# aehogan/lammps-induced-dipole-polarization-pair-style

Measured on AMD Instinct MI355X. Metric: atom-steps/sec, higher is better.
Workload: dtype f64

## Files before the change

lammps-induced-dipole-polarization-pair-style_amd/csrc/lab/api_env_knobs.inc:

```
  if (const char *e = getenv("POLAR_ABLATE")) h->ablate = atoi(e);
  if (const char *e = getenv("POLAR_HOST_COLORS")) h->host_colors = atoi(e) != 0;
  if (const char *e = getenv("POLAR_SWEEP_KERNEL")) h->sweep_kernel = atoi(e);
  if (const char *e = getenv("POLAR_TILE_WAVES")) h->tile_waves = atoi(e) == 8 ? 8 : 4;
  if (const char *e = getenv("POLAR_TILE_WIDE")) h->tile_wide = atoi(e) != 0;
  if (const char *e = getenv("POLAR_CACHE_R2")) h->cache_r2 = atoi(e);
  if (const char *e = getenv("POLAR_LJ_TYPED")) h->lj_typed = atoi(e) != 0;
  if (const char *e = getenv("POLAR_STATIC_XQ")) h->static_xq = atoi(e) != 0;
  if (const char *e = getenv("POLAR_POL_FIRST")) h->pol_first = atoi(e) != 0;
  if (const char *e = getenv("POLAR_LP_WG_PER_CU")) h->lp_wg_per_cu = atoi(e);
  if (const char *e = getenv("POLAR_LP_QM")) h->lp_quad_major = atoi(e) != 0;
  if (const char *e = getenv("POLAR_LP_TILES")) h->lp_tiles = atoi(e) == 1 ? 1 : 2;
  if (const char *e = getenv("POLAR_LP_ROWS")) h->lp_rows = std::max(1, std::min(64, atoi(e)));
  if (const char *e = getenv("POLAR_LP_PAIRS")) h->lp_pairs = atoi(e) != 0;
  if (const char *e = getenv("POLAR_CLUSTER_DIST")) h->cluster_dist = atof(e);
  if (const char *e = getenv("POLAR_CLUSTER_MAX")) h->cluster_max = std::max(1, std::min(4, atoi(e)));
  if (const char *e = getenv("POLAR_LP_DEPTH")) { int v = atoi(e); h->lp_depth = (v == 2 || v == 3) ? v : 0; }
  if (const char *e = getenv("POLAR_QUAD_BLOCK")) { int v = atoi(e); if (v >= 64 && v <= 1024 && v % 64 == 0) h->quad_block = v; }
  if (const char *e = getenv("POLAR_FIELD_BLOCK")) { int v = atoi(e); if (v >= 64 && v <= 1024 && v % 64 == 0) h->field_block = v; }
  if (const char *e = getenv("POLAR_FORCE_LITERAL")) h->force_literal = atoi(e) != 0;
```

lammps-induced-dipole-polarization-pair-style_amd/csrc/polar_api.hip:

```cpp
#include "polar_handle.hpp"

namespace {
void upload_types(polar_handle *h, int ntypes, const double *const t[7]) {
  need_device(h);
  const size_t m = (size_t)(ntypes + 1) * (ntypes + 1);
  std::vector<double> pack(8 * m, 0.0);
  for (size_t k = 0; k < m; k++) {
    pack[8 * k + 0] = t[6][k]; pack[8 * k + 1] = t[5][k]; pack[8 * k + 2] = t[0][k]; pack[8 * k + 3] = t[1][k];
    pack[8 * k + 4] = t[2][k]; pack[8 * k + 5] = t[3][k]; pack[8 * k + 6] = t[4][k];
  }
  h->d_lj.ensure(8 * m);
  HIPCHECK(hipMemcpy(h->d_lj.p, pack.data(), 8 * m * sizeof(double), hipMemcpyHostToDevice));
  h->P.ntypes = ntypes;
  h->P.ljpack = h->d_lj.p;
  h->ntypes = ntypes;
  h->types_set = true;
}

void upload_coul(polar_handle *h, double g_ewald, double qqrd2e, const double *slj, const double *scoul, int nbits,
                 int mask, int shift, double tabinnersq, const double *const t[8]) {
  need_device(h);
  h->P.g_ewald = g_ewald; h->P.qqrd2e = qqrd2e;
  for (int k = 0; k < 4; k++) { h->P.special_lj[k] = slj[k]; h->P.special_coul[k] = scoul[k]; }
  h->P.ncoultablebits = nbits; h->P.ncoulmask = mask; h->P.ncoulshiftbits = shift; h->P.tabinnersq = tabinnersq;
// ... 222 lines not shown

const char *polar_last_error(const polar_handle *h) { return h ? h->err.c_str() : "null handle"; }
const char *polar_last_warning(const polar_handle *h) { return h ? h->warn.c_str() : ""; }

int polar_pair_settings(polar_handle *h, int narg, const char *const *arg) {
  return guarded(h, [&]() { h->ph.settings(narg, arg); h->colors_valid = false; h->nl_pitch = h->dd_pitch = 0; h->cl_pitch = 0; h->un_pitch = 0; h->pitch16 = 0; return POLAR_OK; });
}
int polar_pair_coeff(polar_handle *h, int ntypes, int narg, const char *const *arg) {
  return guarded(h, [&]() { h->ph.coeff(ntypes, narg, arg); return POLAR_OK; });
}
int polar_pair_modify(polar_handle *h, int narg, const char *const *arg) {
  return guarded(h, [&]() { h->ph.modify(narg, arg); return POLAR_OK; });
}
int polar_pair_init(polar_handle *h, double g_ewald, double qqrd2e, const double special_lj[4],
                    const double special_coul[4]) {
  return guarded(h, [&]() {
    PairHost &p = h->ph;
    p.init(g_ewald, qqrd2e, special_lj, special_coul);
    h->coul_set = false;
    if (h->have_device) {
      HIPCHECK(hipSetDevice(h->device));
      const double *t[7] = {p.lj1.data(), p.lj2.data(), p.lj3.data(), p.lj4.data(), p.offset.data(), p.cut_ljsq.data(), p.cutsq.data()};
      upload_types(h, p.ntypes, t);
      if (p.ncoultablebits == 0) {
        const double *c[8];
        double dummy = 0.0;
        for (int k = 0; k < 8; k++) c[k] = &dummy;
        upload_coul(h, g_ewald, qqrd2e, special_lj, special_coul, 0, 0, 0, 0.0, c);
      }
    }
    return POLAR_OK;
  });
}
double polar_pair_cut(const polar_handle *h, int i, int j) {
  if (!h || !h->ph.inited || i < 1 || j < 1 || i > h->ph.ntypes || j > h->ph.ntypes) return -1.0;
  return std::sqrt(h->ph.cutsq[(size_t)i * h->ph.w() + j]);
}
double polar_pair_single(const polar_handle *h, double qi, double qj, int itype, int jtype, double rsq,
                         double factor_coul, double factor_lj, double *fforce) {
  double ff = 0.0, e;
  try {
    e = h->ph.single(qi, qj, itype, jtype, rsq, factor_coul, factor_lj, ff);
  } catch (const std::exception &ex) {
    const_cast<polar_handle *>(h)->err = ex.what();
    e = ff = std::nan("");
  }
  if (fforce) *fforce = ff;
  return e;
}
const void *polar_pair_extract(const polar_handle *h, const char *name, int *dim) {
  if (!h || !name) return nullptr;
  if (dim) *dim = 0;
  if (strcmp(name, "cut_coul") == 0) return &h->ph.st.cut_coul;
  if (dim) *dim = 2;
  if (strcmp(name, "epsilon") == 0) return h->ph.epsilon.data();
  if (strcmp(name, "sigma") == 0) return h->ph.sigma.data();
  if (strcmp(name, "cut_lj") == 0) return h->ph.cut_lj.data();
  return nullptr;
}
int polar_get_settings(const polar_handle *h, polar_settings *out) {
  if (!h || !out) return POLAR_ERR_STATE;
  *out = h->ph.st;
  return POLAR_OK;
}
namespace {
const int kRestartMagic = 0x524C4F50;
const int kRestartVersion = 2;
const int kRestartPayloadV1 = 4 * (int)sizeof(double) + 10 * (int)sizeof(int);
const int kRestartPayload = kRestartPayloadV1 + 4 * (int)sizeof(int) + (int)sizeof(double);
}
int polar_restart_pack(const polar_handle *h, void *buf, int max_bytes) {
  if (!h) return POLAR_ERR_STATE;
  const int total = POLAR_RESTART_HEADER_BYTES + kRestartPayload;
  if (!buf) return total;
  if (max_bytes < total) return POLAR_ERR_INPUT;
  const polar_settings &st = h->ph.st;
  char *p = (char *)buf;
  const int head[3] = {kRestartMagic, kRestartVersion, kRestartPayload};
  memcpy(p, head, sizeof(head)); p += sizeof(head);
  const double d[4] = {st.polar_precision, st.polar_damp, st.polar_gamma, st.dd_cutoff};
  memcpy(p, d, sizeof(d)); p += sizeof(d);
  const int iv[10] = {st.iterations_max, st.damping_type, st.zodid, st.fixed_iteration, st.polar_gs, st.polar_gs_ranked,
                      st.use_previous, st.debug, st.device_neigh, st.restart_polar};
  memcpy(p, iv, sizeof(iv)); p += sizeof(iv);
  const int iv2[4] = {st.deterministic, st.rccl_halo, st.polar_accel, 0};
  memcpy(p, iv2, sizeof(iv2)); p += sizeof(iv2);
  memcpy(p, &st.polar_sor, sizeof(double));
  return total;
}
int polar_restart_unpack(polar_handle *h, const void *buf, int nbytes) {
  return guarded(h, [&]() {
    if (!buf || nbytes < POLAR_RESTART_HEADER_BYTES) throw InputError("not a polarization restart record");
    const char *p = (const char *)buf;
    int head[3];
    memcpy(head, p, sizeof(head)); p += sizeof(head);
    if (head[0] != kRestartMagic) throw InputError("not a polarization restart record");
    const bool v1 = head[1] == 1 && head[2] == kRestartPayloadV1, v2 = head[1] == kRestartVersion && head[2] == kRestartPayload;
    if (!(v1 || v2) || nbytes < POLAR_RESTART_HEADER_BYTES + head[2])
      throw InputError("polarization restart record of an unknown version or length");
    double d[4]; int iv[10];
    memcpy(d, p, sizeof(d)); p += sizeof(d);
    memcpy(iv, p, sizeof(iv)); p += sizeof(iv);
    polar_settings s = h->ph.st;
    s.polar_precision = d[0]; s.polar_damp = d[1]; s.polar_gamma = d[2]; s.dd_cutoff = d[3];
    s.iterations_max = iv[0]; s.damping_type = iv[1]; s.zodid = iv[2]; s.fixed_iteration = iv[3]; s.polar_gs = iv[4];
    s.polar_gs_ranked = iv[5]; s.use_previous = iv[6]; s.debug = iv[7]; s.device_neigh = iv[8]; s.restart_polar = iv[9];
// ... 676 lines not shown
```

lammps-induced-dipole-polarization-pair-style_amd/csrc/polar_common.hpp:

```cpp
#pragma once

#include <hip/hip_runtime.h>
#include <stdint.h>

#ifdef POLAR_LAB
#define POLAR_LAB_PARAM , int ablate
#define POLAR_LAB_PASS , ablate
#define POLAR_ABL(bit) (ablate & (bit))
#else
#define POLAR_LAB_PARAM
#define POLAR_LAB_PASS
#define POLAR_ABL(bit) 0
#endif

namespace polar {


struct __attribute__((aligned(64))) AtomRec {
  double x, mx;
  double y, my;
  double z, mz;
  double q, a;
};

// ... 121 lines not shown
__device__ __forceinline__ double quad_xor(double v, const int which) {
  int lo = __double2loint(v), hi = __double2hiint(v);
  if (which == 1) {
    lo = __builtin_amdgcn_update_dpp(0, lo, 0xB1, 0xF, 0xF, true);
    hi = __builtin_amdgcn_update_dpp(0, hi, 0xB1, 0xF, 0xF, true);
  } else {
    lo = __builtin_amdgcn_update_dpp(0, lo, 0x4E, 0xF, 0xF, true);
    hi = __builtin_amdgcn_update_dpp(0, hi, 0x4E, 0xF, 0xF, true);
  }
  return __hiloint2double(hi, lo);
}
__device__ __forceinline__ double quad_sum(double v) {
  v += quad_xor(v, 1);
  v += quad_xor(v, 2);
  return v;
}

struct RowList {
  const int *cnt;
  long long pitch;
};
__device__ __forceinline__ void row_range(const RowList &L, int i, long long &beg, long long &end) {
  beg = (long long)i * L.pitch;
  const long long c = L.cnt[i];
  end = beg + (c < L.pitch ? c : L.pitch);
}

__device__ __forceinline__ void min_image_rint(const Box &b, double xi, double yi, double zi, double xj, double yj,
                                               double zj, double &dx, double &dy, double &dz) {
  double ex = xi - xj, ey = yi - yj, ez = zi - zj;
  const double nz = b.periodic[2] ? rint(ez * b.inv[2]) : 0.0;
  ez = fma(-b.prd[2], nz, ez); ey = fma(-b.yz, nz, ey); ex = fma(-b.xz, nz, ex);
  const double ny = b.periodic[1] ? rint(ey * b.inv[1]) : 0.0;
  ey = fma(-b.prd[1], ny, ey); ex = fma(-b.xy, ny, ex);
  const double nx = b.periodic[0] ? rint(ex * b.inv[0]) : 0.0;
  ex = fma(-b.prd[0], nx, ex);
  dx = ex; dy = ey; dz = ez;
}
template <bool TRI>
__device__ __forceinline__ bool min_image_rint_w(const Box &b, double xi, double yi, double zi, double xj, double yj,
                                                 double zj, double &dx, double &dy, double &dz) {
  double ex = xi - xj, ey = yi - yj, ez = zi - zj;
  const double nz = b.periodic[2] ? rint(ez * b.inv[2]) : 0.0;
  ez = fma(-b.prd[2], nz, ez);
  if (TRI) { ey = fma(-b.yz, nz, ey); ex = fma(-b.xz, nz, ex); }
  const double ny = b.periodic[1] ? rint(ey * b.inv[1]) : 0.0;
  ey = fma(-b.prd[1], ny, ey);
  if (TRI) ex = fma(-b.xy, ny, ex);
  const double nx = b.periodic[0] ? rint(ex * b.inv[0]) : 0.0;
  ex = fma(-b.prd[0], nx, ex);
  dx = ex; dy = ey; dz = ez;
  return nz != 0.0 || ny != 0.0 || nx != 0.0;
}
__host__ __device__ __forceinline__ void frac_coords(const Box &b, const double lo[3], double x, double y, double z, double fr[3]) {
  fr[2] = (z - lo[2]) * b.inv[2];
  if (b.triclinic) {
    fr[1] = ((y - lo[1]) - b.yz * fr[2] * 1.0) * b.inv[1];
    fr[0] = ((x - lo[0]) - b.xy * fr[1] - b.xz * fr[2]) * b.inv[0];
  } else {
    fr[1] = (y - lo[1]) * b.inv[1];
    fr[0] = (x - lo[0]) * b.inv[0];
  }
}
template <bool EXACT>
__device__ __forceinline__ void pair_del(const Box &b, double xi, double yi, double zi, double xj, double yj,
                                         double zj, double &dx, double &dy, double &dz) {
  if (EXACT) min_image_del(b, xi, yi, zi, xj, yj, zj, dx, dy, dz);
  else min_image_rint(b, xi, yi, zi, xj, yj, zj, dx, dy, dz);
}

__host__ __device__ __forceinline__ long long lp_slot(long long e, int qm = 1) {
  const long long p = e & 63;
  const long long lane = qm ? (((p & 15) << 2) | (p >> 4)) : p;
  return ((e >> 8) << 8) + (lane << 2) + ((e >> 6) & 3);
}

#define POLAR_NL_SAMEMOL 0x40000000
#define POLAR_NL_MASK 0x3FFFFFFF

struct RecQuad { double2 a, b, c, d; };
__device__ __forceinline__ RecQuad fetch_records(const AtomRec *__restrict__ rec, int j, double2 *stage, int lane) {
  const int q4 = lane >> 2;
  const char *base = reinterpret_cast<const char *>(rec);
  const unsigned piece = (unsigned)(lane & 3) * 16u, k = lane & 3;
  const unsigned j0 = __shfl(j, q4, 64), j1 = __shfl(j, 16 + q4, 64), j2 = __shfl(j, 32 + q4, 64), j3 = __shfl(j, 48 + q4, 64);
  const double2 p0 = *reinterpret_cast<const double2 *>(base + ((j0 << 6) + piece));
  const double2 p1 = *reinterpret_cast<const double2 *>(base + ((j1 << 6) + piece));
  const double2 p2 = *reinterpret_cast<const double2 *>(base + ((j2 << 6) + piece));
  const double2 p3 = *reinterpret_cast<const double2 *>(base + ((j3 << 6) + piece));
  stage[q4 * 5 + k] = p0; stage[(16 + q4) * 5 + k] = p1;
  stage[(32 + q4) * 5 + k] = p2; stage[(48 + q4) * 5 + k] = p3;
  __builtin_amdgcn_fence(__ATOMIC_RELEASE, "wavefront");
  __builtin_amdgcn_wave_barrier();
  __builtin_amdgcn_fence(__ATOMIC_ACQUIRE, "wavefront");
  RecQuad r;
  r.a = stage[lane * 5]; r.b = stage[lane * 5 + 1]; r.c = stage[lane * 5 + 2]; r.d = stage[lane * 5 + 3];
  __builtin_amdgcn_wave_barrier();
  return r;
}

struct XQ { double2 a, b; };
__device__ __forceinline__ XQ fetch_xq(const double4 *__restrict__ xq, int j, double2 *stage, int lane) {
  const int h2 = lane >> 1;
  const char *base = reinterpret_cast<const char *>(xq);
  const unsigned piece = (unsigned)(lane & 1) * 16u, k = lane & 1;
  const unsigned j0 = __shfl(j, h2, 64), j1 = __shfl(j, 32 + h2, 64);
  const double2 p0 = *reinterpret_cast<const double2 *>(base + ((j0 << 5) + piece));
  const double2 p1 = *reinterpret_cast<const double2 *>(base + ((j1 << 5) + piece));
  stage[h2 * 3 + k] = p0; stage[(32 + h2) * 3 + k] = p1;
  __builtin_amdgcn_fence(__ATOMIC_RELEASE, "wavefront");
  __builtin_amdgcn_wave_barrier();
  __builtin_amdgcn_fence(__ATOMIC_ACQUIRE, "wavefront");
  XQ r;
  r.a = stage[lane * 3]; r.b = stage[lane * 3 + 1];
  __builtin_amdgcn_wave_barrier();
  return r;
}

struct ExpCoef {
  double log2e, ln2hi, ln2lo;
  double c[14];
};
inline ExpCoef make_expcoef() {
  ExpCoef K;
  K.log2e = 1.4426950408889634074; K.ln2hi = 6.93147180369123816490e-01; K.ln2lo = 1.90821492927058770002e-10;
  const double c[14] = {1.0, 1.0, 0.5, 0.16666666666666666, 0.041666666666666664, 0.008333333333333333, 0.001388888888888889, 0.0001984126984126984, 2.48015873015873e-05, 2.7557319223985893e-06, 2.755731922398589e-07, 2.505210838544172e-08, 2.08767569878681e-09, 1.6059043836821613e-10};
  for (int k = 0; k < 14; k++) K.c[k] = c[k];
// ... 91 lines not shown
```

lammps-induced-dipole-polarization-pair-style_amd/csrc/polar_handle.hpp:

```cpp
#pragma once
#include <hip/hip_runtime.h>

#include <algorithm>
#include <initializer_list>
#include <utility>
#include <chrono>
#include <cmath>
#include <cstdio>
#include <cstdlib>
#include <exception>
#include <cstring>
#include <numeric>
#include <string>
#include <thread>
#include <mutex>
#include <condition_variable>
#include <functional>
#include <memory>
#include <stdexcept>
#include <unistd.h>
#include <vector>

#include "pair_host.hpp"
#include "polar_kernels.hpp"
// ... 145 lines not shown
  DBuf<double> d_mu0;
  bool mu0_saved = false;
  int attempt = 0;
  int last_sweeps = 0;
  bool mu_host_in_sync = false;
  std::vector<int> color_off;
  std::vector<int> color_sub;
  int color_nsub = 1;
  DBuf<int> d_bflag; int bflag_n = 0;
  std::vector<int *> h_nl_stage; std::vector<hipEvent_t> ev_nl;
  hipStream_t up_stream = nullptr; hipEvent_t ev_list_up = nullptr; bool list_up_pending = false;
  std::vector<long long> h_first; std::vector<int> h_nn, h_ilist;
  bool colors_global = false;
  std::vector<int> user_colors;
  bool user_colors_clashed = false;
  std::vector<int> h_rows;
  bool colors_valid = false;
  double color_keep = 2.0;
  bool slots_by_color = false;
  long long color_epoch = 0;
  long long slots_epoch = -1;
  bool colors_recheck = false;
  std::vector<int> h_color;
  DBuf<int> d_color_orig, d_color_s;
  DBuf<int> d_klist;
  DBuf<int> d_cadj, d_cdeg, d_ccnt, d_cflags, d_crelabel;
  DBuf<unsigned long long> d_cprio;
  DBuf<double> d_cstat;
  DBuf<long long> d_coff;
  int *h_cflags = nullptr;
  double *h_cstat = nullptr;
  long long *h_coff = nullptr;
  int cadj_pitch = 16;
  int host_colors = 0;
  int colors_reused = 0, colors_rebuilt = 0;
  double ms_color_host = 0.0;
  double color_dist = 2.4;
  int field_block = 256;
  double bbox_lo[3] = {0, 0, 0}, bbox_hi[3] = {0, 0, 0};
  long long global_count = 0;
  DBuf<double> d_xchg; DBuf<int> d_xidx;
  bool device_list = false;
  int user_full_list = 0;
  long long lj_pitch = 0;
  DBuf<double4> d_ljpos; DBuf<int2> d_ljaux; DBuf<int> d_tag, d_nspecial, d_special, d_ljcell_id, d_ljcell_cnt, d_ljcell_fill; DBuf<long long> d_ljcell_first; DBuf<double> d_cutneighsq;
  int lj_typed = 1;
  bool lj_tab_arith = false;
  int lj_pers = 1;
  int ncu = 0;
  int lj_pers_threads = 768;
  bool sym_typed = false, dev_typed = false;
  int static_xq = 1;
  int pol_first = 1;
#ifdef POLAR_LAB
  int force_literal = 0;
#endif
  int part_k = 0, part_n = 1;
  int lp_wg_per_cu = 0;
  int lp_quad_major = 1;
  int quad_block = POLAR_BLOCK;
  int lp_tiles = 2;
  int lp_rows = 1;
  int lp_pairs = 0;
  DBuf<int> d_ulead, d_udd_j;
  DBuf<long long> d_upos;
  DBuf<int2> d_unit;
  DBuf<int4> d_udesc;
  std::vector<int> unit_off;
  long long upitch = 0;
  int lp_depth = 0;
  int cache_r2 = -1;
  int stream_mode = 1;
  int sweep_kernel = 2;
  int ablate = 0;
  DBuf<SRec> d_srec0, d_srec1;
  DBuf<TileHdr> d_thdr;
  DBuf<TileRowEnt> d_trow;
  DBuf<int> d_un_j;
  DBuf<unsigned short> d_dd16;
  DBuf<double> d_pend;
  int un_pitch = 0;
  int un_lds = 0;
  long long pitch16 = 0;
  int tile_max_u = 0;
  bool tile_reported = false;
  double dens = 0.0;
  std::vector<TileLaunch> tile_launches;
  TileLaunch tile_all{};
  size_t tile_lds_attr[16] = {0, 0, 0, 0, 0, 0, 0, 0, 0, 0, 0, 0, 0, 0, 0, 0};
  size_t tile_build_lds_attr = 0;
  int tile_waves = 4;
  int tile_wide = 0;
  int tile_sw[3] = {2, 2, 2};
  int deterministic = 0;
  Scal *h_scal = nullptr;
  hipEvent_t ev[8] = {};
  hipStream_t lj_stream = nullptr;
  hipEvent_t ev_fork = nullptr, ev_join = nullptr, ev_lj0 = nullptr, ev_lj1 = nullptr, ev_dl0 = nullptr, ev_dl1 = nullptr;
  hipStream_t dl_stream = nullptr;
  hipEvent_t ev_mu_ready = nullptr;
  double *early_mu = nullptr, *early_ef = nullptr, *user_mu = nullptr, *user_ef = nullptr;
  hipEvent_t ev_fchunk[4] = {nullptr, nullptr, nullptr, nullptr};
  bool overlap_lj = true;
  bool lj_forked = false;
  std::vector<double> h_tmp;
  double *h_stage = nullptr;
  DBuf<double> d_trace;
// ... 198 lines not shown
```

lammps-induced-dipole-polarization-pair-style_amd/csrc/polar_lists.hpp:

```cpp
#pragma once

#include "polar_common.hpp"

namespace polar {

struct CellGrid {
  int trim;
  int nc[3];
  double lo[3], inv[3];
};

__device__ __forceinline__ int cell_of(const CellGrid &g, const Box &b, double x, double y, double z) {
  int c[3];
  double fr3[3];
  frac_coords(b, g.lo, x, y, z, fr3);
#pragma unroll
  for (int k = 0; k < 3; k++) {
    double fr = fr3[k];
    fr -= floor(fr);
    int ck = (int)(fr * g.nc[k]);
    c[k] = ck >= g.nc[k] ? g.nc[k] - 1 : ck;
  }
  return (c[2] * g.nc[1] + c[1]) * g.nc[0] + c[0];
}

static __global__ void k_cell_count(int n, const double *__restrict__ x, CellGrid g, Box b, int *__restrict__ cell_id,
                             int *__restrict__ cell_cnt) {
  int i = blockIdx.x * blockDim.x + threadIdx.x;
  if (i >= n) return;
  int c = cell_of(g, b, x[3 * i], x[3 * i + 1], x[3 * i + 2]);
  cell_id[i] = c;
  atomicAdd(&cell_cnt[c], 1);
}

#define POLAR_SCAN_ITEMS 4096
static __global__ __launch_bounds__(1024) void k_scan_block(long long n, const int *__restrict__ in, long long *__restrict__ out,
                                                     long long *__restrict__ btot) {
  __shared__ long long wtot[16];
  const int t = threadIdx.x, lane = t & 63, wv = t >> 6;
  const long long base = (long long)blockIdx.x * POLAR_SCAN_ITEMS + 4 * t;
  int v[4] = {0, 0, 0, 0};
  if (base + 3 < n) { const int4 q = *(const int4 *)(in + base); v[0] = q.x; v[1] = q.y; v[2] = q.z; v[3] = q.w; }
  else for (int k = 0; k < 4; k++) if (base + k < n) v[k] = in[base + k];
  const long long s = (long long)v[0] + v[1] + v[2] + v[3];
  long long inc = s;
#pragma unroll
  for (int off = 1; off < 64; off <<= 1) {
    const long long up = __shfl_up(inc, off, 64);
    if (lane >= off) inc += up;
  }
  if (lane == 63) wtot[wv] = inc;
  __syncthreads();
  if (wv == 0) {
    long long x = lane < 16 ? wtot[lane] : 0, w = x;
#pragma unroll
// ... 362 lines not shown
  __shared__ double part[128];
  if (threadIdx.x < 128) part[threadIdx.x] = 0.0;
  __syncthreads();
  const int i = blockIdx.x * blockDim.x + threadIdx.x;
  int c = i < n ? color_s[i] : -1;
  if (c >= 0) { const int o = perm[i]; if (o < own_lo || o >= own_hi) c = -1; }
  if (c >= 0) {
    atomicAdd(&part[2 * c], 1.0);
    atomicAdd(&part[2 * c + 1], rank ? rank[i] : 1.0);
  }
  __syncthreads();
  if (threadIdx.x < 128 && part[threadIdx.x] != 0.0) atomicAdd(sums + threadIdx.x, part[threadIdx.x]);
}
static __global__ void k_color_relabel(int n, const int *__restrict__ relabel, const int *__restrict__ perm, int *__restrict__ color_s,
                                int *__restrict__ color_orig) {
  const int i = blockIdx.x * blockDim.x + threadIdx.x;
  if (i >= n) return;
  const int c = color_s[i] >= 0 ? relabel[color_s[i]] : -1;
  color_s[i] = c;
  color_orig[perm[i]] = c;
}
__device__ __forceinline__ int color_class(int j, const int *__restrict__ color_s, const int *__restrict__ perm, int own_lo, int own_hi,
                                           const int *__restrict__ sub, int nsub) {
  const int c = color_s[j];
  if (c < 0) return -1;
  const int o = perm[j];
  if (o < own_lo || o >= own_hi) return -1;
  return sub ? nsub * c + sub[o] : c;
}
static __global__ void k_color_cellcount(long long ncell, int nclass, const long long *__restrict__ cell_first, const int *__restrict__ npol,
                                  const int *__restrict__ color_s, int *__restrict__ cnt, const int *__restrict__ perm, int own_lo, int own_hi,
                                  const int *__restrict__ sub, int nsub) {
  const long long c = blockIdx.x * (long long)blockDim.x + threadIdx.x;
  if (c >= ncell) return;
  const int a = (int)cell_first[c], e = a + npol[c];
  for (int q = 0; q < nclass; q++) {
    int k = 0;
    for (int j = a; j < e; j++) k += color_class(j, color_s, perm, own_lo, own_hi, sub, nsub) == q;
    cnt[(size_t)q * ncell + c] = k;
  }
}
static __global__ void k_color_fill(long long ncell, int nclass, const long long *__restrict__ cell_first, const int *__restrict__ npol,
                             const int *__restrict__ color_s, const int *__restrict__ perm, const long long *__restrict__ off,
                             int *__restrict__ rows_orig, int own_lo, int own_hi, const int *__restrict__ sub, int nsub) {
  const long long c = blockIdx.x * (long long)blockDim.x + threadIdx.x;
  if (c >= ncell) return;
  const int a = (int)cell_first[c], e = a + npol[c];
  for (int q = 0; q < nclass; q++) {
    long long w = off[(size_t)q * ncell + c];
    for (int j = a; j < e; j++) if (color_class(j, color_s, perm, own_lo, own_hi, sub, nsub) == q) rows_orig[w++] = perm[j];
  }
}

template <bool TRI, bool RECHECK>
static __global__ __launch_bounds__(POLAR_BLOCK) void k_nl_build(const int *__restrict__ rows, int nrows,
                                                          const double4 *__restrict__ pos4, Box box, CellGrid g,
                                                          const long long *__restrict__ cell_first, double cutallsq,
                                                          double ddcutsq, long long nl_pitch, long long dd_pitch,
                                                          int *__restrict__ nl_cnt, int *__restrict__ dd_cnt,
                                                          int *__restrict__ nl_j, int *__restrict__ dd_j,
                                                          double *__restrict__ dd_r2, int pad_dd,
                                                          int dd_shift_qm, int dd_pad_index, int *__restrict__ dd_wrap,
                                                          const int *__restrict__ color_s, double colordistsq,
                                                          int *__restrict__ color_conflict,
                                                          const int *__restrict__ dd_slot,
                                                          int *__restrict__ overflow,
                                                          unsigned long long *__restrict__ dd_total) {
  const int dd_shift = dd_shift_qm & 255, dd_qm = dd_shift_qm >> 8;
  const int lane = threadIdx.x & 63;
  const int row = blockIdx.x * POLAR_ROWS_PER_BLOCK + (threadIdx.x >> 6);
  if (row >= nrows) return;
  const int i = rows ? rows[row] : row;
  const double4 ri = pos4[i];
  const int imol = __double2hiint(ri.w), ipol = __double2loint(ri.w);
  const int icol = (RECHECK && color_s && ipol) ? color_s[i] : -2;
  bool clash = RECHECK && color_s && ipol && icol < 0;
  int cc[3];
  double uu[3], edge[3];
  {
    double fr3[3];
    frac_coords(box, g.lo, ri.x, ri.y, ri.z, fr3);
#pragma unroll
    for (int k = 0; k < 3; k++) {
      double fr = fr3[k];
      fr -= floor(fr);
      const double t = fr * g.nc[k];
      int ck = (int)t;
      ck = ck >= g.nc[k] ? g.nc[k] - 1 : ck;
      cc[k] = __builtin_amdgcn_readfirstlane(ck);
      uu[k] = wave_uniform(t - ck); edge[k] = wave_uniform(box.prd[k] / g.nc[k]);
    }
  }
  const int c0 = cc[0], c1 = cc[1], c2 = cc[2];
  const int slot_i = dd_slot ? dd_slot[i] : i;
  const long long nl0 = (long long)i * nl_pitch, dd0 = (long long)(slot_i >= 0 ? slot_i : 0) * dd_pitch;
  int ncount = 0, dcount = 0;
  bool wrap_lane = false;
  const unsigned long long below = (lane == 0) ? 0ull : (~0ull >> (64 - lane));
  const int n0 = g.nc[0], n1 = g.nc[1], n2 = g.nc[2];
  const int zlo = n2 >= 5 ? c2 - 2 : 0, zcnt = n2 >= 5 ? 5 : n2;
  const int ylo = n1 >= 5 ? c1 - 2 : 0, ycnt = n1 >= 5 ? 5 : n1;
  const double reach = sqrt(cutallsq > ddcutsq ? cutallsq : ddcutsq) + 1e-6;
  const double reach2 = wave_uniform(reach * reach);
  const int nsr = zcnt * ycnt;
  int ra0 = 0, rb0 = 0, ra1 = 0, rb1 = 0;
  if (lane < nsr) {
    const int zz = zlo + lane / ycnt, yy = ylo + lane % ycnt;
    int b2 = zz, b1 = yy;
    bool ok = true;
    if (b2 < 0 || b2 >= n2) { if (!box.periodic[2]) ok = false; b2 = (b2 + n2) % n2; }
    if (b1 < 0 || b1 >= n1) { if (!box.periodic[1]) ok = false; b1 = (b1 + n1) % n1; }
    double dzmin = 0.0, dymin = 0.0;
    if (n2 >= 5) { const int d = zz - c2; dzmin = d > 0 ? (d - uu[2]) * edge[2] : (d < 0 ? (uu[2] - (d + 1)) * edge[2] : 0.0); }
    if (n1 >= 5) { const int d = yy - c1; dymin = d > 0 ? (d - uu[1]) * edge[1] : (d < 0 ? (uu[1] - (d + 1)) * edge[1] : 0.0); }
    const double rem2 = reach2 - dzmin * dzmin - dymin * dymin;
    if (g.trim && rem2 < 0.0) ok = false;
    int xlo = n0 >= 5 ? c0 - 2 : 0, xhi = n0 >= 5 ? c0 + 2 : n0 - 1;
    if (ok && g.trim && n0 >= 5) {
      const double xr = sqrt(rem2) / edge[0];
      int lo_off = (int)floor(uu[0] - xr), hi_off = (int)floor(uu[0] + xr);
      lo_off = lo_off < -2 ? -2 : lo_off; hi_off = hi_off > 2 ? 2 : hi_off;
      xlo = c0 + lo_off; xhi = c0 + hi_off;
    }
    if (ok) {
      const long long rowbase = ((long long)b2 * n1 + b1) * n0;
      const int xa = xlo < 0 ? 0 : xlo, xb = xhi >= n0 ? n0 - 1 : xhi;
      ra0 = (int)cell_first[rowbase + xa]; rb0 = (int)cell_first[rowbase + xb + 1];
      if (box.periodic[0]) {
        if (xlo < 0) { ra1 = (int)cell_first[rowbase + xlo + n0]; rb1 = (int)cell_first[rowbase + n0]; }
        else if (xhi >= n0) { ra1 = (int)cell_first[rowbase]; rb1 = (int)cell_first[rowbase + xhi - n0 + 1]; }
      }
    }
  }
  for (int sr = 0; sr < nsr; sr++) {
#pragma unroll
    for (int piece = 0; piece < 2; piece++) {
      const int a = __builtin_amdgcn_readlane(piece ? ra1 : ra0, sr), b = __builtin_amdgcn_readlane(piece ? rb1 : rb0, sr);
      for (int base = a; base < b; base += 64) {
        const int p = base + lane;
        bool in_nl = false, in_dd = false;
        const int j = p;
        int same = 0;
        double rsq = 0.0;
        if (p < b && j != i) {
          const double4 rj = pos4[j];
          double ex, ey, ez;
          const bool shifted = min_image_rint_w<TRI>(box, ri.x, ri.y, ri.z, rj.x, rj.y, rj.z, ex, ey, ez);
          rsq = ex * ex + ey * ey + ez * ez;
          in_nl = rsq <= cutallsq;
          in_dd = ipol && slot_i >= 0 && __double2loint(rj.w) && (rsq < ddcutsq);
          if (RECHECK && icol >= 0 && rsq < colordistsq && __double2loint(rj.w) && color_s[j] == icol) clash = true;
          wrap_lane |= in_dd && shifted;
          same = (imol != 0 && imol == __double2hiint(rj.w)) ? POLAR_NL_SAMEMOL : 0;
        }
        const unsigned long long m_nl = __ballot(in_nl), m_dd = __ballot(in_dd);
        const int kn = ncount + __popcll(m_nl & below), kd = dcount + __popcll(m_dd & below);
        if (in_nl && kn < nl_pitch) nl_j[nl0 + kn] = j | same;
        if (in_dd && kd < dd_pitch) {
          dd_j[dd0 + (dd_shift ? lp_slot(kd, dd_qm) : (long long)kd)] = j << dd_shift;
          if (dd_r2) dd_r2[dd0 + kd] = rsq;
        }
        ncount += __popcll(m_nl);
        dcount += __popcll(m_dd);
      }
    }
  }
  if (pad_dd) {
    const int have = dcount < dd_pitch ? dcount : (int)dd_pitch;
    const int padded = (have + 63) & ~63;
    for (int k = have + lane; k < padded; k += 64) {
      dd_j[dd0 + (dd_shift ? lp_slot(k, dd_qm) : (long long)k)] = (dd_pad_index >= 0 ? dd_pad_index : i) << dd_shift;
      if (dd_r2) dd_r2[dd0 + k] = 1e60;
    }
  }
  if (RECHECK && color_s && __ballot(clash) != 0ull && lane == 0) atomicOr(color_conflict, 1);
  const unsigned long long anywrap = __ballot(wrap_lane);
  if (lane == 0) {
    nl_cnt[i] = ncount; dd_cnt[i] = dcount;
    if (dd_wrap) dd_wrap[i] = anywrap != 0ull;
    if (ncount > nl_pitch || dcount > dd_pitch) atomicMax(overflow, ncount > dcount ? ncount : dcount);
    if (dcount) atomicAdd(dd_total + (blockIdx.x & 63) * 16, (unsigned long long)(dcount < dd_pitch ? dcount : (int)dd_pitch));
  }
}

#ifdef POLAR_LAB
#include "lab/lists_paired_rows.hpp"
#endif

#ifdef POLAR_LAB
#include "lab/lists_cluster_rows.hpp"
#endif

struct LJGrid {
  int nc[3];
  double lo[3], inv[3];
};
__device__ __forceinline__ int lj_cell_of(const LJGrid &g, double x, double y, double z) {
  const double p[3] = {x, y, z};
  int c[3];
#pragma unroll
  for (int k = 0; k < 3; k++) {
    int ck = (int)floor((p[k] - g.lo[k]) * g.inv[k]);
    c[k] = ck < 0 ? 0 : (ck >= g.nc[k] ? g.nc[k] - 1 : ck);
  }
  return (c[2] * g.nc[1] + c[1]) * g.nc[0] + c[0];
}
static __global__ void k_lj_cell_count(int nall, const double *__restrict__ x, LJGrid g, int *__restrict__ cell_id,
                                int *__restrict__ cell_cnt) {
  int i = blockIdx.x * blockDim.x + threadIdx.x;
  if (i >= nall) return;
  const int c = lj_cell_of(g, x[3 * i], x[3 * i + 1], x[3 * i + 2]);
  cell_id[i] = c;
  atomicAdd(&cell_cnt[c], 1);
}
static __global__ void k_lj_cell_fill(int nall, const int *__restrict__ cell_id, const long long *__restrict__ cell_first,
                               int *__restrict__ fill, const double *__restrict__ x, const int *__restrict__ type,
                               const int *__restrict__ mol, const int *__restrict__ tag, double4 *__restrict__ pos,
                               int2 *__restrict__ aux) {
  int i = blockIdx.x * blockDim.x + threadIdx.x;
  if (i >= nall) return;
  const int c = cell_id[i];
  const int s = (int)cell_first[c] + atomicAdd(&fill[c], 1);
  pos[s] = make_double4(x[3 * i], x[3 * i + 1], x[3 * i + 2], __hiloint2double(mol[i], type[i]));
  aux[s] = make_int2(i, tag ? tag[i] : i + 1);
}

static __global__ __launch_bounds__(POLAR_BLOCK) void k_lj_nl_build(int row_lo, int nrows, int ntypes, const double *__restrict__ x,
                                                             const int *__restrict__ type, const int *__restrict__ mol,
                                                             const double4 *__restrict__ pos, const int2 *__restrict__ aux,
                                                             LJGrid g, const long long *__restrict__ cell_first,
                                                             const double *__restrict__ cutneighsq, Box box,
                                                             int exclude_intra, const int *__restrict__ nspecial,
// ... 200 lines not shown
```

lammps-induced-dipole-polarization-pair-style_amd/csrc/polar_step.hip:

```cpp
#include "polar_handle.hpp"

void launch_scan(long long n, const int *in, long long *out, DBuf<long long> &tot, hipStream_t s) {
  const int nb = (int)std::max<long long>(1, (n + POLAR_SCAN_ITEMS - 1) / POLAR_SCAN_ITEMS);
  tot.ensure((size_t)nb + 1);
  k_scan_block<<<nb, 1024, 0, s>>>(n, in, out, tot.p);
  if (nb > 1) {
    k_scan_totals<<<1, 1024, 0, s>>>(nb, tot.p, out + n);
    k_scan_add<<<nblk(n - POLAR_SCAN_ITEMS, 256), 256, 0, s>>>(n, out, tot.p);
  }
}

void build_cells(polar_handle *h) {
  const polar_settings &st = h->ph.st;
  const int n = h->nlocal;
  const double cutall = std::max(st.cut_coul, st.dd_cutoff);
  double width[3];
  box_widths(h->box, width);
  for (int k = 0; k < 3; k++)
    if (h->box.periodic[k] && width[k] < 2.0 * cutall * (1.0 - 1e-12))
      throw InputError("dd_cutoff mode needs box lengths >= 2*max(cut_coul,dd_cutoff); use exact mode (dd_cutoff 0)");
  CellGrid &g = h->grid;
  g.trim = 1;
#ifdef POLAR_LAB
  if (const char *e = getenv("POLAR_NL_TRIM")) g.trim = atoi(e);
// ... 86 lines not shown
          double fr = (h->hx[3 * (size_t)a + k] - h->grid.lo[k]) / h->box.prd[k];
          fr -= std::floor(fr);
          c += mul * std::min(nc[k] - 1, (int)(fr * nc[k]));
          mul *= nc[k];
        }
        occ[(size_t)c] = 1;
      }
      long long filled = 0;
      for (char v : occ) filled += v;
      if (filled > 0) vol *= (double)filled / (double)tot;
    }
    h->dens = n / vol;
    double mean = n / vol * 4.18879020478639 * cutall * cutall * cutall;
    h->nl_pitch = h->dd_pitch = (((long long)(1.5 * mean) + 64) / 64 + 1) * 64;
  }
  if (h->sweep_kernel == 2) h->dd_pitch = ((h->dd_pitch + 255) / 256) * 256;
  if ((h->sweep_kernel == 2 || h->sweep_kernel == 3) && ((long long)n + 1) * (long long)sizeof(AtomRec) >= (1ll << 31))
    throw InputError("more than 2^25 atoms on one handle: the 32-bit record offsets of the sweep's index stream would wrap (shard the system)");
  h->d_nl_cnt.ensure(n + 1); h->d_dd_cnt.ensure(n + 1);
  h->d_nl_j.ensure((size_t)n * h->nl_pitch + 64);
  if (h->sweep_kernel < 3) h->d_dd_j.ensure((size_t)n * h->dd_pitch + 1024);
  else h->d_dd_j.ensure(64);
  int mode = h->cache_r2;
  if (h->sweep_kernel == 1) mode = 0;
  if (h->sweep_kernel == 2) mode = 3;
  if (h->sweep_kernel >= 3) mode = 4;
  if (mode < 0) {
    const double est_pairs = h->dd_pairs > 0 ? (double)h->dd_pairs : 0.35 * (double)own_n(h) * (double)h->dd_pitch;
    mode = (12.0 * est_pairs < 200.0e6) ? 1 : 2;
  }
  h->stream_mode = mode;
  const bool r2c = mode == 1;
  if (mode == 1) h->d_dd_r2.ensure((size_t)n * h->dd_pitch + 64);
  else if (mode == 0) h->d_dd_s.ensure((size_t)n * h->dd_pitch + 64);
  double *r2p = r2c ? h->d_dd_r2.p : nullptr;
  double2 *sp = mode == 0 ? h->d_dd_s.p : nullptr;
  bool fuse = mode != 0 && mode != 4;
#ifdef POLAR_LAB
  if (getenv("POLAR_NO_FUSE_R2")) fuse = false;
#endif
  const double cutallsq = cutall * cutall, ddsq = mode == 4 ? -1.0 : st.dd_cutoff * st.dd_cutoff;
  const int nr = own_n(h);
  const int *rows = own_rows(h);
  zero_many(s, {{h->d_nl_cnt.p, (size_t)(n + 1) * sizeof(int)}, {h->d_dd_cnt.p, (size_t)(n + 1) * sizeof(int)},
                {h->d_overflow.p, 16 * sizeof(int)}, {h->d_ddtot.p, 64 * 16 * sizeof(unsigned long long)}});
  const bool lp = mode == 3;
  if (lp) h->d_dd_wrap.ensure(n + 1);
  const bool recheck = h->colors_valid && h->colors_recheck && h->sweep_kernel < 3 && (int)h->h_color.size() == n;
  if (h->colors_recheck && !recheck) { h->colors_valid = false; h->colors_recheck = false; }
  if (recheck) {
    h->d_color_s.ensure(n + 1);
    k_color_map<<<nblk(n, 256), 256, 0, s>>>(n, h->d_perm.p, h->d_color_orig.p, h->d_color_s.p);
  }
#define NLB(TRI, RC)                                                                                                          \
  k_nl_build<TRI, RC><<<nblk(nr, POLAR_ROWS_PER_BLOCK), POLAR_BLOCK, 0, s>>>(                                                 \
      rows, nr, h->d_pos4.p, h->box, g, h->d_cell_first.p, cutallsq, ddsq, h->nl_pitch, h->dd_pitch, h->d_nl_cnt.p,            \
      h->d_dd_cnt.p, h->d_nl_j.p, h->d_dd_j.p, fuse ? r2p : nullptr, fuse ? 1 : 0, lp ? (6 | (h->lp_quad_major << 8)) : 0,    \
      lp ? n : -1, lp ? h->d_dd_wrap.p : nullptr, recheck ? h->d_color_s.p : nullptr, h->color_keep * h->color_keep,           \
      h->d_overflow.p + 8, lp ? h->d_slot.p : nullptr, h->d_overflow.p, h->d_ddtot.p)
  if (h->box.triclinic) { if (recheck) NLB(true, true); else NLB(true, false); }
  else                  { if (recheck) NLB(false, true); else NLB(false, false); }
#undef NLB
  const RowList ddl{h->d_dd_cnt.p, h->dd_pitch};
  if (fuse || mode == 4) {
  }
#ifdef POLAR_LAB
  else if (st.damping_type == POLAR_DAMP_EXPONENTIAL)
    k_dd_scalars<0><<<nblk(nr, POLAR_ROWS_PER_BLOCK), POLAR_BLOCK, 0, s>>>(rows, nr, h->d_rec0.p, h->box, ddl, h->d_dd_j.p, st.polar_damp, sp, r2p);
  else
    k_dd_scalars<1><<<nblk(nr, POLAR_ROWS_PER_BLOCK), POLAR_BLOCK, 0, s>>>(rows, nr, h->d_rec0.p, h->box, ddl, h->d_dd_j.p, st.polar_damp, sp, r2p);
#endif
  HIPCHECK(hipMemcpyAsync(h->h_flags, h->d_overflow.p, sizeof(int), hipMemcpyDeviceToHost, s));
  HIPCHECK(hipMemcpyAsync(h->h_ddtot, h->d_ddtot.p, 64 * 16 * sizeof(unsigned long long), hipMemcpyDeviceToHost, s));
}
template <bool AP>
static void launch_rank(polar_handle *h, int pass) {
  const int n = h->nlocal, ntot = h->nlocal + h->nghost;
  dim3 grid(nblk(n, POLAR_ROWS_PER_BLOCK)), block(POLAR_BLOCK);
  if (pass == 2) k_fold_scal<<<1, POLAR_NSLOT, 0, h->stream>>>(h->d_scal.p, h->d_slots.p, 1);
  const int nchunk = (AP && pass == 1) ? std::max(1, std::min(16, 8192 / std::max(n, 1))) : 1;
  if (pass == 1)
    k_rank<AP, 1><<<nblk((long long)n * nchunk, POLAR_ROWS_PER_BLOCK), block, 0, h->stream>>>(n, ntot, h->d_x.p, h->d_alpha.p, h->d_mol.p, h->box, RowList{h->d_nl_cnt.p, h->nl_pitch},
                                                 h->d_nl_j.p, h->d_rec0.p, h->d_mol_s.p, h->d_scal.p, h->d_slots.p, h->d_rank.p, nchunk);
  else
    k_rank<AP, 2><<<grid, block, 0, h->stream>>>(n, ntot, h->d_x.p, h->d_alpha.p, h->d_mol.p, h->box, RowList{h->d_nl_cnt.p, h->nl_pitch},
                                                 h->d_nl_j.p, h->d_rec0.p, h->d_mol_s.p, h->d_scal.p, h->d_slots.p, h->d_rank.p, 1);
}

void launch_rank_pass(polar_handle *h, bool allpairs, int pass) {
  if (allpairs) launch_rank<true>(h, pass); else launch_rank<false>(h, pass);
}

template <bool AP, int DAMP, int EP>
void launch_field(polar_handle *h, int nrows, const int *rows) {
  const polar_settings &st = h->ph.st;
  if (nrows <= 0) return;
  const int fb = h->field_block;
  const size_t lds = AP ? 0 : (size_t)(fb / 64) * 64 * 5 * sizeof(double2);
  k_field<AP, DAMP, EP><<<nblk(nrows, fb / 64), fb, lds, h->stream>>>(
      nrows, rows, h->nlocal, h->d_rec0.p, h->d_rec1.p, h->box, RowList{h->d_dd_cnt.p, h->dd_pitch}, h->d_dd_j.p, h->d_dd_s.p,
      st.dd_cutoff * st.dd_cutoff, st.polar_damp, h->d_ef_s.p, h->d_F.p, h->d_scal.p, h->d_slots.p
#ifdef POLAR_LAB
      , h->ablate
#endif
      );
}
template <int EP>
void launch_field_dyn(polar_handle *h, bool ap, int nrows, const int *rows) {
  const bool expd = h->ph.st.damping_type == POLAR_DAMP_EXPONENTIAL;
  if (ap) { if (expd) launch_field<true, 0, EP>(h, nrows, rows); else launch_field<true, 1, EP>(h, nrows, rows); }
#ifdef POLAR_LAB
  else    { if (expd) launch_field<false, 0, EP>(h, nrows, rows); else launch_field<false, 1, EP>(h, nrows, rows); }
#else
  else throw std::logic_error("k_field's list branch exists in the lab build only");
#endif
// ... 840 lines not shown
```

Baseline: 15.69 million.

## Pack neighbor-list candidate cell runs densely across wave lanes

The neighbor-list build kernel now concatenates all candidate cell ranges of a row into one dense index space using a DPP prefix sum. Each 64-lane sweep covers candidates from several cells instead of padding each cell range to full waves. The per-candidate work is also rewritten with ballots, mbcnt prefix counts, 32-bit byte offsets, readfirstlane on row indices, and a branch-free periodic image. This is meant to cut idle lanes in the list build, at the cost of a per-sweep shift lookup over the run table and a new 2^27-atom limit.

```diff
diff --git a/lammps-induced-dipole-polarization-pair-style_amd/csrc/lab/api_env_knobs.inc b/lammps-induced-dipole-polarization-pair-style_amd/csrc/lab/api_env_knobs.inc
--- a/lammps-induced-dipole-polarization-pair-style_amd/csrc/lab/api_env_knobs.inc
+++ b/lammps-induced-dipole-polarization-pair-style_amd/csrc/lab/api_env_knobs.inc
@@ -18,3 +18,4 @@
   if (const char *e = getenv("POLAR_QUAD_BLOCK")) { int v = atoi(e); if (v >= 64 && v <= 1024 && v % 64 == 0) h->quad_block = v; }
   if (const char *e = getenv("POLAR_FIELD_BLOCK")) { int v = atoi(e); if (v >= 64 && v <= 1024 && v % 64 == 0) h->field_block = v; }
   if (const char *e = getenv("POLAR_FORCE_LITERAL")) h->force_literal = atoi(e) != 0;
+  if (const char *e = getenv("POLAR_NL_DENSE")) h->nl_dense = atoi(e) != 0;
diff --git a/lammps-induced-dipole-polarization-pair-style_amd/csrc/polar_api.hip b/lammps-induced-dipole-polarization-pair-style_amd/csrc/polar_api.hip
--- a/lammps-induced-dipole-polarization-pair-style_amd/csrc/polar_api.hip
+++ b/lammps-induced-dipole-polarization-pair-style_amd/csrc/polar_api.hip
@@ -298,6 +298,7 @@
   if (!h || !name) return nullptr;
   if (dim) *dim = 0;
   if (strcmp(name, "cut_coul") == 0) return &h->ph.st.cut_coul;
+  if (strcmp(name, "nl_dense") == 0) return &h->nl_dense_used;
   if (dim) *dim = 2;
   if (strcmp(name, "epsilon") == 0) return h->ph.epsilon.data();
   if (strcmp(name, "sigma") == 0) return h->ph.sigma.data();
diff --git a/lammps-induced-dipole-polarization-pair-style_amd/csrc/polar_common.hpp b/lammps-induced-dipole-polarization-pair-style_amd/csrc/polar_common.hpp
--- a/lammps-induced-dipole-polarization-pair-style_amd/csrc/polar_common.hpp
+++ b/lammps-induced-dipole-polarization-pair-style_amd/csrc/polar_common.hpp
@@ -197,6 +197,21 @@
   dx = ex; dy = ey; dz = ez;
   return nz != 0.0 || ny != 0.0 || nx != 0.0;
 }
+template <bool TRI>
+__device__ __forceinline__ unsigned long long min_image_rint_m(const Box &b, double xi, double yi, double zi, double xj, double yj,
+                                                               double zj, double &dx, double &dy, double &dz) {
+  double ex = xi - xj, ey = yi - yj, ez = zi - zj;
+  const double nz = rint(ez * b.inv[2]);
+  ez = fma(-b.prd[2], nz, ez);
+  if (TRI) { ey = fma(-b.yz, nz, ey); ex = fma(-b.xz, nz, ex); }
+  const double ny = rint(ey * b.inv[1]);
+  ey = fma(-b.prd[1], ny, ey);
+  if (TRI) ex = fma(-b.xy, ny, ex);
+  const double nx = rint(ex * b.inv[0]);
+  ex = fma(-b.prd[0], nx, ex);
+  dx = ex; dy = ey; dz = ez;
+  return __builtin_amdgcn_ballot_w64(nz != 0.0) | __builtin_amdgcn_ballot_w64(ny != 0.0) | __builtin_amdgcn_ballot_w64(nx != 0.0);
+}
 __host__ __device__ __forceinline__ void frac_coords(const Box &b, const double lo[3], double x, double y, double z, double fr[3]) {
   fr[2] = (z - lo[2]) * b.inv[2];
   if (b.triclinic) {
@@ -218,6 +233,11 @@
   const long long p = e & 63;
   const long long lane = qm ? (((p & 15) << 2) | (p >> 4)) : p;
   return ((e >> 8) << 8) + (lane << 2) + ((e >> 6) & 3);
+}
+__host__ __device__ __forceinline__ unsigned lp_slot32(unsigned e, int qm) {
+  const unsigned p = e & 63u;
+  const unsigned lane = qm ? (((p & 15u) << 2) | (p >> 4)) : p;
+  return (e & ~255u) + (lane << 2) + ((e >> 6) & 3u);
 }
 
 #define POLAR_NL_SAMEMOL 0x40000000
diff --git a/lammps-induced-dipole-polarization-pair-style_amd/csrc/polar_handle.hpp b/lammps-induced-dipole-polarization-pair-style_amd/csrc/polar_handle.hpp
--- a/lammps-induced-dipole-polarization-pair-style_amd/csrc/polar_handle.hpp
+++ b/lammps-induced-dipole-polarization-pair-style_amd/csrc/polar_handle.hpp
@@ -221,7 +221,9 @@
   bool sym_typed = false, dev_typed = false;
   int static_xq = 1;
   int pol_first = 1;
+  double nl_dense_used = 1.0;
 #ifdef POLAR_LAB
+  int nl_dense = 1;
   int force_literal = 0;
 #endif
   int part_k = 0, part_n = 1;
diff --git a/lammps-induced-dipole-polarization-pair-style_amd/csrc/polar_lists.hpp b/lammps-induced-dipole-polarization-pair-style_amd/csrc/polar_lists.hpp
--- a/lammps-induced-dipole-polarization-pair-style_amd/csrc/polar_lists.hpp
+++ b/lammps-induced-dipole-polarization-pair-style_amd/csrc/polar_lists.hpp
@@ -1,6 +1,7 @@
 #pragma once
 
 #include "polar_common.hpp"
+#include "polar_nl_dense.hpp"
 
 namespace polar {
 
@@ -469,7 +470,20 @@
   }
 }
 
-template <bool TRI, bool RECHECK>
+__device__ __forceinline__ int prefix_count(unsigned long long m, int base) {
+  return __builtin_amdgcn_mbcnt_hi((unsigned)(m >> 32), __builtin_amdgcn_mbcnt_lo((unsigned)m, base));
+}
+struct NlRunLanes {
+  int s0v, k0v, s1v, k1v, endv;
+  unsigned m1;
+  __device__ __forceinline__ int s0(int sr) const { return __builtin_amdgcn_readlane(s0v, sr); }
+  __device__ __forceinline__ int k0(int sr) const { return __builtin_amdgcn_readlane(k0v, sr); }
+  __device__ __forceinline__ int s1(int sr) const { return __builtin_amdgcn_readlane(s1v, sr); }
+  __device__ __forceinline__ int k1(int sr) const { return __builtin_amdgcn_readlane(k1v, sr); }
+  __device__ __forceinline__ int end(int sr) const { return __builtin_amdgcn_readlane(endv, sr); }
+  __device__ __forceinline__ bool two(int sr) const { return (m1 >> sr) & 1u; }
+};
+template <bool TRI, bool RECHECK, bool DENSE = true>
 static __global__ __launch_bounds__(POLAR_BLOCK) void k_nl_build(const int *__restrict__ rows, int nrows,
                                                           const double4 *__restrict__ pos4, Box box, CellGrid g,
                                                           const long long *__restrict__ cell_first, double cutallsq,
@@ -487,7 +501,7 @@
   const int lane = threadIdx.x & 63;
   const int row = blockIdx.x * POLAR_ROWS_PER_BLOCK + (threadIdx.x >> 6);
   if (row >= nrows) return;
-  const int i = rows ? rows[row] : row;
+  const int i = __builtin_amdgcn_readfirstlane(rows ? rows[row] : row);
   const double4 ri = pos4[i];
   const int imol = __double2hiint(ri.w), ipol = __double2loint(ri.w);
   const int icol = (RECHECK && color_s && ipol) ? color_s[i] : -2;
@@ -509,10 +523,19 @@
     }
   }
   const int c0 = cc[0], c1 = cc[1], c2 = cc[2];
-  const int slot_i = dd_slot ? dd_slot[i] : i;
+  const int slot_i = __builtin_amdgcn_readfirstlane(dd_slot ? dd_slot[i] : i);
   const long long nl0 = (long long)i * nl_pitch, dd0 = (long long)(slot_i >= 0 ? slot_i : 0) * dd_pitch;
+  char *const nl_row = reinterpret_cast<char *>(nl_j + nl0), *const dd_row = reinterpret_cast<char *>(dd_j + dd0);
+  char *const r2_row = reinterpret_cast<char *>(dd_r2 ? dd_r2 + dd0 : nullptr);
+  const char *const pos_b = reinterpret_cast<const char *>(pos4);
+  const int nl_cap = (int)nl_pitch, dd_cap = (int)dd_pitch;
+  const unsigned long long dd_im = (ipol && slot_i >= 0) ? ~0ull : 0ull;
+  Box pbox = box;
+#pragma unroll
+  for (int k = 0; k < 3; k++) { pbox.inv[k] = box.periodic[k] ? box.inv[k] : 0.0; pbox.periodic[k] = 1; }
   int ncount = 0, dcount = 0;
-  bool wrap_lane = false;
+  unsigned long long wrap_m = 0ull;
+  const int same_i = imol != 0 ? POLAR_NL_SAMEMOL : 0;
   const unsigned long long below = (lane == 0) ? 0ull : (~0ull >> (64 - lane));
   const int n0 = g.nc[0], n1 = g.nc[1], n2 = g.nc[2];
   const int zlo = n2 >= 5 ? c2 - 2 : 0, zcnt = n2 >= 5 ? 5 : n2;
@@ -522,11 +545,12 @@
   const int nsr = zcnt * ycnt;
   int ra0 = 0, rb0 = 0, ra1 = 0, rb1 = 0;
   if (lane < nsr) {
-    const int zz = zlo + lane / ycnt, yy = ylo + lane % ycnt;
+    const int lz = (lane >= ycnt) + (lane >= 2 * ycnt) + (lane >= 3 * ycnt) + (lane >= 4 * ycnt);
+    const int zz = zlo + lz, yy = ylo + (lane - lz * ycnt);
     int b2 = zz, b1 = yy;
     bool ok = true;
-    if (b2 < 0 || b2 >= n2) { if (!box.periodic[2]) ok = false; b2 = (b2 + n2) % n2; }
-    if (b1 < 0 || b1 >= n1) { if (!box.periodic[1]) ok = false; b1 = (b1 + n1) % n1; }
+    if (b2 < 0 || b2 >= n2) { if (!box.periodic[2]) ok = false; b2 = b2 < 0 ? b2 + n2 : b2 - n2; }
+    if (b1 < 0 || b1 >= n1) { if (!box.periodic[1]) ok = false; b1 = b1 < 0 ? b1 + n1 : b1 - n1; }
     double dzmin = 0.0, dymin = 0.0;
     if (n2 >= 5) { const int d = zz - c2; dzmin = d > 0 ? (d - uu[2]) * edge[2] : (d < 0 ? (uu[2] - (d + 1)) * edge[2] : 0.0); }
     if (n1 >= 5) { const int d = yy - c1; dymin = d > 0 ? (d - uu[1]) * edge[1] : (d < 0 ? (uu[1] - (d + 1)) * edge[1] : 0.0); }
@@ -549,36 +573,55 @@
       }
     }
   }
-  for (int sr = 0; sr < nsr; sr++) {
-#pragma unroll
-    for (int piece = 0; piece < 2; piece++) {
-      const int a = __builtin_amdgcn_readlane(piece ? ra1 : ra0, sr), b = __builtin_amdgcn_readlane(piece ? rb1 : rb0, sr);
-      for (int base = a; base < b; base += 64) {
-        const int p = base + lane;
-        bool in_nl = false, in_dd = false;
-        const int j = p;
-        int same = 0;
-        double rsq = 0.0;
-        if (p < b && j != i) {
-          const double4 rj = pos4[j];
-          double ex, ey, ez;
-          const bool shifted = min_image_rint_w<TRI>(box, ri.x, ri.y, ri.z, rj.x, rj.y, rj.z, ex, ey, ez);
-          rsq = ex * ex + ey * ey + ez * ez;
-          in_nl = rsq <= cutallsq;
-          in_dd = ipol && slot_i >= 0 && __double2loint(rj.w) && (rsq < ddcutsq);
-          if (RECHECK && icol >= 0 && rsq < colordistsq && __double2loint(rj.w) && color_s[j] == icol) clash = true;
-          wrap_lane |= in_dd && shifted;
-          same = (imol != 0 && imol == __double2hiint(rj.w)) ? POLAR_NL_SAMEMOL : 0;
-        }
-        const unsigned long long m_nl = __ballot(in_nl), m_dd = __ballot(in_dd);
-        const int kn = ncount + __popcll(m_nl & below), kd = dcount + __popcll(m_dd & below);
-        if (in_nl && kn < nl_pitch) nl_j[nl0 + kn] = j | same;
-        if (in_dd && kd < dd_pitch) {
-          dd_j[dd0 + (dd_shift ? lp_slot(kd, dd_qm) : (long long)kd)] = j << dd_shift;
-          if (dd_r2) dd_r2[dd0 + kd] = rsq;
-        }
-        ncount += __popcll(m_nl);
-        dcount += __popcll(m_dd);
+  auto candidate = [&](const int p, const bool valid) {
+    const int j = valid ? p : i;
+    const double4 rj = *reinterpret_cast<const double4 *>(pos_b + ((unsigned)j << 5));
+    double ex, ey, ez;
+    const unsigned long long shifted = min_image_rint_m<TRI>(pbox, ri.x, ri.y, ri.z, rj.x, rj.y, rj.z, ex, ey, ez);
+    const double rsq = ex * ex + ey * ey + ez * ez;
+    const unsigned long long m_pair = __builtin_amdgcn_ballot_w64(j != i);
+    const unsigned long long m_nl = m_pair & __builtin_amdgcn_ballot_w64(rsq <= cutallsq);
+    const unsigned long long m_dd = m_pair & dd_im & __builtin_amdgcn_ballot_w64(__double2loint(rj.w) != 0) & __builtin_amdgcn_ballot_w64(rsq < ddcutsq);
+    wrap_m |= m_dd & shifted;
+    const bool in_nl = (j != i) & (rsq <= cutallsq);
+    const bool in_dd = (j != i) & (dd_im != 0ull) & (__double2loint(rj.w) != 0) & (rsq < ddcutsq);
+    if (RECHECK) { if (icol >= 0 && j != i && rsq < colordistsq && __double2loint(rj.w) != 0 && color_s[j] == icol) clash = true; }
+    int jmol = __double2hiint(rj.w);
+    asm("" : "+v"(jmol));
+    const int same = imol == jmol ? same_i : 0;
+    const int kn = prefix_count(m_nl, ncount), kd = prefix_count(m_dd, dcount);
+    if (in_nl && kn < nl_cap) *reinterpret_cast<int *>(nl_row + ((unsigned)kn << 2)) = j | same;
+    if (in_dd && kd < dd_cap) {
+      *reinterpret_cast<int *>(dd_row + ((dd_shift ? lp_slot32((unsigned)kd, dd_qm) : (unsigned)kd) << 2)) = j << dd_shift;
+      if (dd_r2) *reinterpret_cast<double *>(r2_row + ((unsigned)kd << 3)) = rsq;
+    }
+    ncount += __popcll(m_nl);
+    dcount += __popcll(m_dd);
+  };
+  if (DENSE) {
+    const int len = nl_run_len(ra0, rb0, ra1, rb1);
+    int inc = len;
+    inc += __builtin_amdgcn_update_dpp(0, inc, 0x111, 0xF, 0xF, true);
+    inc += __builtin_amdgcn_update_dpp(0, inc, 0x112, 0xF, 0xF, true);
+    inc += __builtin_amdgcn_update_dpp(0, inc, 0x114, 0xF, 0xF, true);
+    inc += __builtin_amdgcn_update_dpp(0, inc, 0x118, 0xF, 0xF, true);
+    const int row0 = __builtin_amdgcn_readlane(inc, 15);
+    inc += (lane >= 16 && lane < 32) ? row0 : 0;
+    const int total = __builtin_amdgcn_readlane(inc, 31);
+    const NlRunEntry e = nl_run_entry(ra0, rb0, ra1, rb1, inc - len);
+    const NlRunLanes tab{e.s0, e.k0, e.s1, e.k1, e.end, (unsigned)__ballot(rb1 > ra1)};
+    unsigned rem = (unsigned)__ballot(len > 0);
+    for (int t0 = 0; t0 < total; t0 += 64) {
+      const int g = t0 + lane;
+      const int k = nl_dense_shift(tab, rem, t0, g);
+      candidate(g + k, g < total);
+    }
+  } else {
+    for (int sr = 0; sr < nsr; sr++) {
+#pragma unroll
+      for (int piece = 0; piece < 2; piece++) {
+        const int a = __builtin_amdgcn_readlane(piece ? ra1 : ra0, sr), b = __builtin_amdgcn_readlane(piece ? rb1 : rb0, sr);
+        for (int base = a; base < b; base += 64) candidate(base + lane, base + lane < b);
       }
     }
   }
@@ -591,10 +634,9 @@
     }
   }
   if (RECHECK && color_s && __ballot(clash) != 0ull && lane == 0) atomicOr(color_conflict, 1);
-  const unsigned long long anywrap = __ballot(wrap_lane);
   if (lane == 0) {
     nl_cnt[i] = ncount; dd_cnt[i] = dcount;
-    if (dd_wrap) dd_wrap[i] = anywrap != 0ull;
+    if (dd_wrap) dd_wrap[i] = wrap_m != 0ull;
     if (ncount > nl_pitch || dcount > dd_pitch) atomicMax(overflow, ncount > dcount ? ncount : dcount);
     if (dcount) atomicAdd(dd_total + (blockIdx.x & 63) * 16, (unsigned long long)(dcount < dd_pitch ? dcount : (int)dd_pitch));
   }
diff --git a/lammps-induced-dipole-polarization-pair-style_amd/csrc/polar_nl_dense.hpp b/lammps-induced-dipole-polarization-pair-style_amd/csrc/polar_nl_dense.hpp
--- /dev/null
+++ b/lammps-induced-dipole-polarization-pair-style_amd/csrc/polar_nl_dense.hpp
@@ -0,0 +1,42 @@
+#pragma once
+
+#if defined(__HIPCC__)
+#define POLAR_NLD_FN __host__ __device__ __forceinline__
+#else
+#define POLAR_NLD_FN inline
+#endif
+
+namespace polar {
+
+struct NlRunEntry {
+  int s0, k0, s1, k1, end;
+};
+POLAR_NLD_FN int nl_run_len(int ra0, int rb0, int ra1, int rb1) {
+  return (rb0 > ra0 ? rb0 - ra0 : 0) + (rb1 > ra1 ? rb1 - ra1 : 0);
+}
+POLAR_NLD_FN NlRunEntry nl_run_entry(int ra0, int rb0, int ra1, int rb1, int off) {
+  NlRunEntry e;
+  const int len0 = rb0 > ra0 ? rb0 - ra0 : 0, len1 = rb1 > ra1 ? rb1 - ra1 : 0;
+  e.s0 = off; e.k0 = ra0 - off;
+  e.s1 = off + len0; e.k1 = ra1 - e.s1;
+  e.end = e.s1 + len1;
+  return e;
+}
+template <class Tab>
+POLAR_NLD_FN int nl_dense_shift(const Tab &tab, unsigned &rem, int t0, int g) {
+  int k = 0;
+  while (rem) {
+    const int sr = __builtin_ctz(rem);
+    const int s0 = tab.s0(sr), k0 = tab.k0(sr);
+    k = g >= s0 ? k0 : k;
+    if (tab.two(sr)) {
+      const int s1 = tab.s1(sr), k1 = tab.k1(sr);
+      k = g >= s1 ? k1 : k;
+    }
+    if (tab.end(sr) > t0 + 64) break;
+    rem &= rem - 1;
+  }
+  return k;
+}
+
+}
diff --git a/lammps-induced-dipole-polarization-pair-style_amd/csrc/polar_step.hip b/lammps-induced-dipole-polarization-pair-style_amd/csrc/polar_step.hip
--- a/lammps-induced-dipole-polarization-pair-style_amd/csrc/polar_step.hip
+++ b/lammps-induced-dipole-polarization-pair-style_amd/csrc/polar_step.hip
@@ -162,15 +162,24 @@
     h->d_color_s.ensure(n + 1);
     k_color_map<<<nblk(n, 256), 256, 0, s>>>(n, h->d_perm.p, h->d_color_orig.p, h->d_color_s.p);
   }
-#define NLB(TRI, RC)                                                                                                          \
-  k_nl_build<TRI, RC><<<nblk(nr, POLAR_ROWS_PER_BLOCK), POLAR_BLOCK, 0, s>>>(                                                 \
+  if (((long long)n + 1) * (long long)sizeof(double4) >= (1ll << 32))
+    throw InputError("more than 2^27 atoms on one handle: the 32-bit position offsets of the list build would wrap (shard the system)");
+#define NLB3(TRI, RC, DENSE)                                                                                                  \
+  k_nl_build<TRI, RC, DENSE><<<nblk(nr, POLAR_ROWS_PER_BLOCK), POLAR_BLOCK, 0, s>>>(                                          \
       rows, nr, h->d_pos4.p, h->box, g, h->d_cell_first.p, cutallsq, ddsq, h->nl_pitch, h->dd_pitch, h->d_nl_cnt.p,            \
       h->d_dd_cnt.p, h->d_nl_j.p, h->d_dd_j.p, fuse ? r2p : nullptr, fuse ? 1 : 0, lp ? (6 | (h->lp_quad_major << 8)) : 0,    \
       lp ? n : -1, lp ? h->d_dd_wrap.p : nullptr, recheck ? h->d_color_s.p : nullptr, h->color_keep * h->color_keep,           \
       h->d_overflow.p + 8, lp ? h->d_slot.p : nullptr, h->d_overflow.p, h->d_ddtot.p)
+#ifdef POLAR_LAB
+#define NLB(TRI, RC) do { if (h->nl_dense) NLB3(TRI, RC, true); else NLB3(TRI, RC, false); } while (0)
+  h->nl_dense_used = h->nl_dense ? 1.0 : 0.0;
+#else
+#define NLB(TRI, RC) NLB3(TRI, RC, true)
+#endif
   if (h->box.triclinic) { if (recheck) NLB(true, true); else NLB(true, false); }
   else                  { if (recheck) NLB(false, true); else NLB(false, false); }
 #undef NLB
+#undef NLB3
   const RowList ddl{h->d_dd_cnt.p, h->dd_pitch};
   if (fuse || mode == 4) {
   }
```

After: 15.92 million, median of 6. +1.5%, better.
